# skokec/DAU-ConvNet

Measured on AMD Instinct MI355X. Metric: DAU fwd+bwd GSamples/s (N*H*W/s), higher is better.
Workload: dtype f32

## Files before the change

### dau-convnet_amd/csrc/dau_tiled.hpp

```cpp
#pragma once
#include "dau_common.hpp"

namespace dau {

struct TiledConfig {
    int N, Cin, Cout, G, H, W;
    int R;
    int blur_k;
    int NP;
    int windows;
    int stack;
    int patches;
    int rows, pitch;
    int tiles_x, tiles_y;
    int tile_w;
    int fblock;
    int variant;
    int debug;
    int act;
};

bool tiled_gather_configure(int N, int Cin, int Cout, int G, int H, int W, int R, int blur_k, int act, TiledConfig* cfg);
size_t tiled_gather_workspace_bytes(const TiledConfig& cfg);
int tiled_gather_windows(const TiledConfig& cfg);
// ... 10 lines not shown
    int ftiles;
};
#define DAU_DECLARE_DENSE_GATHER(NS)                                                                                           \
    namespace NS {                                                                                                            \
    bool dense_gather_configure(int N, int Cin, int Cout, int G, int H, int W, int R, int blur_k, int act, DenseConfig* cfg);  \
    size_t dense_gather_workspace_bytes(const DenseConfig& cfg);                                                              \
    void dense_gather_init(const DenseConfig& cfg);                                                                           \
      \
    void dense_gather_prepare(hipStream_t st, const DenseConfig& cfg, const float* in, const float* filters, bool mirrored,   \
                              const UnitRef* table, void* workspace, const Guard& guard);                                     \
    void dense_gather_run(hipStream_t st, const DenseConfig& cfg, float* out, void* workspace, const Guard& guard);           \
    }
DAU_DECLARE_DENSE_GATHER(r4)
DAU_DECLARE_DENSE_GATHER(r3)

#define DAU_DECLARE_SPLIT_GATHER(NS)                                                                                           \
    namespace NS {                                                                                                            \
    bool split_gather_configure(int N, int Cin, int Cout, int G, int H, int W, int R, int blur_k, int act, DenseConfig* cfg);  \
    size_t split_gather_workspace_bytes(const DenseConfig& cfg);                                                              \
    void split_gather_init(const DenseConfig& cfg);                                                                           \
    void split_gather_prepare(hipStream_t st, const DenseConfig& cfg, const float* in, const float* filters, bool mirrored,   \
                              const UnitRef* table, void* workspace, const Guard& guard);                                     \
    void split_gather_run(hipStream_t st, const DenseConfig& cfg, float* out, void* workspace, const Guard& guard);           \
    }
DAU_DECLARE_SPLIT_GATHER(s2)
DAU_DECLARE_SPLIT_GATHER(s3)
DAU_DECLARE_SPLIT_GATHER(s4)

struct TiledDotConfig {
    Shape sh;
    int R, blur_k;
    int NP;
    int variant;
    int windows;
    bool as1, one_tile;
    bool rw8;
    bool ring;
    int region_cols, region_rows;
    int rounds;
    int act;
    int ignore;
    int debug;
};

bool tiled_dot_configure(const Shape& sh, int R, int blur_k, int act, int ignore, TiledDotConfig* cfg);
size_t tiled_dot_workspace_bytes(const TiledDotConfig& cfg);
void tiled_dot_prepare(hipStream_t st, const TiledDotConfig& cfg, const float* x, const float* dy,
                       const float* filters, const UnitRef* table_bare, int drop_col, int drop_row, void* workspace,
                       const Guard& guard);
void tiled_dot_run(hipStream_t st, const TiledDotConfig& cfg, float* r4, void* workspace, const Guard& guard, bool accumulate);
void tiled_dot_init(const TiledDotConfig& cfg);

void launch_blur4_pack(hipStream_t st, const float* x, const float* filters, int N, int C, int cstride, int H, int W, int Hp,
                       int Wp, int blur_k, int act, float* xk, const Guard& guard);
void blur4_pack_init(int blur_k);
bool blur4_pack_fits(int blur_k, int Hp, int Wp);

void launch_dot_reduce(hipStream_t st, const void* partial, int partial_f32, long n, int G, int F, int g_split, int slabs0,
                       int slabs1, int zero_from, bool accumulate, float* r4, const Guard& guard);

struct SplitDotConfig {
    Shape sh;
    int blur_k;
    int RW;
    int act;
};
bool split_dot_configure(const Shape& sh, int blur_k, int act, SplitDotConfig* cfg);
size_t split_dot_workspace_bytes(const SplitDotConfig& cfg);
void split_dot_init(const SplitDotConfig& cfg);
void split_dot_prepare(hipStream_t st, const SplitDotConfig& cfg, const float* x, const float* dy, const float* filters,
                       int drop_col, int drop_row, void* workspace, const Guard& guard);
void split_dot_run(hipStream_t st, const SplitDotConfig& cfg, const UnitRef* table, float* r4, void* workspace, const Guard& guard);

struct WgradConfig {
    Shape sh;
    int blur_k;
    int SB, FB, NC;
    int HsT, WsT, WT, nseg;
    int splits;
    int Hp, Wp;
    bool fused;
};
#define DAU_DECLARE_DENSE_WGRAD(NS)                                                                                            \
    namespace NS {                                                                                                            \
    bool dense_wgrad_configure(const Shape& sh, int blur_k, bool bf16, WgradConfig* cfg);                                     \
    size_t dense_wgrad_workspace_bytes(const WgradConfig& cfg);                                                               \
    void dense_wgrad_init(const WgradConfig& cfg);                                                                            \
    void dense_wgrad_run(hipStream_t st, const WgradConfig& cfg, const float* x, const float* dy, const float* filters,       \
                         const UnitRef* table, int drop_col, int drop_row, float* r4, void* workspace, const Guard& guard, int nk); \
    }
DAU_DECLARE_DENSE_WGRAD(r4)
DAU_DECLARE_DENSE_WGRAD(r3)

}
```

### dau-convnet_amd/csrc/k_gather_dot.hip

```cpp
#include <cstdlib>
#include <algorithm>
#ifndef DAU_DOT_FLUSH_TERMS
#define DAU_DOT_FLUSH_TERMS 1024
#endif
#include <type_traits>
#include <utility>

#include "dau_tiled.hpp"

namespace dau {

typedef float f2 __attribute__((ext_vector_type(2)));
typedef float f4 __attribute__((ext_vector_type(4)));
typedef float f8 __attribute__((ext_vector_type(8)));
typedef float f16 __attribute__((ext_vector_type(16)));
typedef __attribute__((address_space(3))) void* lds_ptr_t;
typedef __attribute__((address_space(1))) const void* glb_ptr_t;

namespace {

constexpr int kDF = 32;
constexpr int kRW = 8;
#ifndef DAU_DOT_WAVES
#define DAU_DOT_WAVES 16
// ... 127 lines not shown
    const int nxc = (EX + kPackErrorChunk - 1) / kPackErrorChunk;
    int t0 = blockIdx.x;
    const int xc = t0 % nxc; t0 /= nxc;
    const int Y = t0 % EY; t0 /= EY;
    const int fb = t0 % nfb;
    const int np = t0 / nfb;
    const int y = Y - (R + 1);
    const int X0 = xc * kPackErrorChunk, X1 = X0 + kPackErrorChunk < EX ? X0 + kPackErrorChunk : EX;
    const int xa0 = X0 - (R + 1) > 0 ? X0 - (R + 1) : 0, xa1 = X1 - (R + 1) < W ? X1 - (R + 1) : W;
    const int cw = xa1 > xa0 ? xa1 - xa0 : 0;
    const int wp = (cw > 0 ? cw : 1) | 1;
    const bool rowin = y >= 0 && y < H && !(drop_row && y == H - 1);
    if (rowin && cw > 0) {
        auto fill = [&](auto actc) {
            constexpr int AF = decltype(actc)::value;
            const int total = 64 * cw;
            for (int t0 = threadIdx.x; t0 < total; t0 += blockDim.x * kLoadBatch) {
                typename RawAct<AF>::type v[kLoadBatch];
                int rr[kLoadBatch];
                bool okk[kLoadBatch];
#pragma unroll
                for (int u = 0; u < kLoadBatch; ++u) {
                    const int t = t0 + u * blockDim.x, tc = t < total ? t : total - 1;
                    const int r = tc / cw, x = tc - r * cw;
                    rr[u] = r;
                    const int f = fb * kDF + (r >> 1), n = 2 * np + (r & 1);
                    const bool ok = f < F && n < N;
                    const long src = (((long)(ok ? n : 0) * F + (ok ? f : 0)) * H + y) * W + xa0;
                    v[u] = load_raw<AF>(dy, src + x);
                    okk[u] = ok;
                }
#pragma unroll
                for (int u = 0; u < kLoadBatch; ++u) {
                    const int t = t0 + u * blockDim.x;
                    if (t < total) lds[rr[u] * wp + (t - rr[u] * cw)] = mask_act(act_of(v[u]), okk[u]);
                }
            }
        };
        with_act(act, fill);
    }
    __syncthreads();
    float* out = ep + ((((size_t)np * nfb + fb) * EY + Y) * EX + X0) * (kDF * 2);
    const int wlim = drop_col ? W - 1 : W;
    for (int t = threadIdx.x; t < (X1 - X0) * 64; t += blockDim.x) {
        const int X = X0 + (t >> 6), r = t & 63, x = X - (R + 1);
        out[t] = (rowin && x >= xa0 && x < xa1 && x < wlim) ? lds[r * wp + (x - xa0)] : 0.0f;
    }
}

struct Blur4Args {
    const float* in;
    const float* taps;
    float* xk;
    int N, C, cstride, H, W, k, Hp, Wp;
    int act;
    int ppb, items;
    unsigned lds_item_floats;
    int WY, WX, nwy, nwx;
    Guard guard;
};

template <int K>
__global__ void __launch_bounds__(512) blur4_pack_kernel(const Blur4Args a) {
    extern __shared__ __attribute__((aligned(16))) float lds[];
    if (!guard_pass(a.guard)) return;
    const int C = a.cstride, H = a.H, W = a.W, k = K ? K : a.k;
    const int Creal = a.C;
    const int lane = threadIdx.x & 63;
    const int nw = (blockDim.x >> 6) / a.ppb;
    const int sub = (threadIdx.x >> 6) / nw, wave = (threadIdx.x >> 6) % nw;
    int t = blockIdx.x * a.ppb + sub;
    const bool active = t < a.items;
    if (!active) t = a.items - 1;
    const int c = t % C; t /= C;
    const int wx = t % a.nwx; t /= a.nwx;
    const int wy = t % a.nwy;
    const int np = t / a.nwy;
    const int oy0 = wy * a.WY, ox0 = wx * a.WX;
    const int oh = oy0 + a.WY < a.Hp ? a.WY : a.Hp - oy0, ow = ox0 + a.WX < a.Wp ? a.WX : a.Wp - ox0;
    const int kr = (k - 1) / 2;
    const int lw = ow + 2 * kr, lh = oh + 2 * kr;
    f2* A = reinterpret_cast<f2*>(lds + (size_t)sub * a.lds_item_floats);
    f2* B = A + (size_t)lh * lw;
    const float* tp[6] = {a.taps + kTapGX * kTapPitch, a.taps + kTapAX * kTapPitch, a.taps + kTapCX * kTapPitch,
                          a.taps + kTapGY * kTapPitch, a.taps + kTapAY * kTapPitch, a.taps + kTapBY * kTapPitch};
    float tr[6][K ? K : 1];
    if (K) {
#pragma unroll
        for (int q = 0; q < 6; ++q)
#pragma unroll
            for (int i = 0; i < K; ++i) tr[q][i] = tp[q][i];
    }
    auto tap = [&](int q, int i) { return K ? tr[q][i] : tp[q][i]; };
    const int n0 = 2 * np, n1 = 2 * np + 1;
    const bool real = c < Creal;
    const int cs = real ? c : 0;
    const long p0 = ((long)n0 * Creal + cs) * H * W, p1 = ((long)(n1 < a.N ? n1 : n0) * Creal + cs) * H * W;
    const float m0 = real ? 1.0f : 0.0f;
    const float m1 = (real && n1 < a.N) ? 1.0f : 0.0f;
    auto for_each = [&](int rows_, int cols_, auto&& body) {
        if (cols_ >= 56) {
            for (int r = wave; r < rows_; r += nw)
                for (int x = lane; x < cols_; x += 64) body(r, x);
        } else {
            for (int t = wave * 64 + lane; t < rows_ * cols_; t += nw * 64) { const int r = t / cols_; body(r, t - r * cols_); }
        }
    };
    auto fill = [&](auto actc) {
        constexpr int AF = decltype(actc)::value;
        struct Raw2 { typename RawAct<AF>::type v0, v1; };
        load_phase<Raw2>(lh, lw, wave, nw, lane,
            [&](int r, int xl) {
                const int yy = oy0 - kr + r, xx = ox0 - kr + xl;
                const bool in = yy >= 0 && yy < H && xx >= 0 && xx < W;
                const long off = in ? (long)yy * W + xx : 0;
                return Raw2{load_raw<AF>(a.in, p0 + off), load_raw<AF>(a.in, p1 + off)};
            },
            [&](int r, int xl, Raw2 v) {
                const int yy = oy0 - kr + r, xx = ox0 - kr + xl;
                const bool in = yy >= 0 && yy < H && xx >= 0 && xx < W;
                A[r * lw + xl] = f2{mask_act(m0 * act_of(v.v0), in), mask_act(m1 * act_of(v.v1), in)};
            });
    };
    with_act(a.act, fill);
    __syncthreads();
    for_each(lh, ow, [&](int r, int x) {
        const int yy = oy0 - kr + r;
        f2 h1 = {0.0f, 0.0f}, h2 = {0.0f, 0.0f}, h3 = {0.0f, 0.0f};
        if (yy >= 0 && yy < H) {
#pragma unroll
            for (int i = 0; i < k; ++i) {
                const f2 v = A[r * lw + x + i];
                h1 = __builtin_elementwise_fma(v, f2{tap(0, i), tap(0, i)}, h1);
                h2 = __builtin_elementwise_fma(v, f2{tap(1, i), tap(1, i)}, h2);
                h3 = __builtin_elementwise_fma(v, f2{tap(2, i), tap(2, i)}, h3);
            }
        }
        B[(0 * lh + r) * ow + x] = h1; B[(1 * lh + r) * ow + x] = h2; B[(2 * lh + r) * ow + x] = h3;
    });
    __syncthreads();
    f8* out = reinterpret_cast<f8*>(a.xk) + ((size_t)np * a.cstride + c) * a.Hp * a.Wp;
    for_each(active ? oh : 0, ow, [&](int yr, int xc) {
        const int yy = oy0 + yr, xx = ox0 + xc;
        f2 dw = {0.0f, 0.0f}, d1 = {0.0f, 0.0f}, d2 = {0.0f, 0.0f}, ds = {0.0f, 0.0f};
        if (yy < H && xx < W) {
#pragma unroll
            for (int j = 0; j < k; ++j) {
                const f2 b1 = B[(0 * lh + yr + j) * ow + xc], b2 = B[(1 * lh + yr + j) * ow + xc], b3 = B[(2 * lh + yr + j) * ow + xc];
                dw = __builtin_elementwise_fma(b1, f2{tap(3, j), tap(3, j)}, dw);
                d1 = __builtin_elementwise_fma(b2, f2{tap(3, j), tap(3, j)}, d1);
                d2 = __builtin_elementwise_fma(b1, f2{tap(4, j), tap(4, j)}, d2);
                ds = __builtin_elementwise_fma(b3, f2{tap(3, j), tap(3, j)}, ds);
                ds = __builtin_elementwise_fma(b1, f2{tap(5, j), tap(5, j)}, ds);
            }
        }
        out[(size_t)yy * a.Wp + xx] = f8{dw.x, dw.y, d1.x, d1.y, d2.x, d2.y, ds.x, ds.y};
    });
}

__global__ void dot_params_kernel(const UnitRef* __restrict__ table, int S, int G, int F, int R, int Rt, int nsub1,
                                  int epitch, int g_begin, int GP, int ngb, int nfb, int s_pad, float* __restrict__ params,
                                  const Guard guard) {
    if (!guard_pass(guard)) return;
    const long total = (long)nsub1 * nsub1 * s_pad * ngb * GP * nfb * 64;
    for (long idx = blockIdx.x * (long)blockDim.x + threadIdx.x; idx < total; idx += (long)gridDim.x * blockDim.x) {
        const int lane = (int)(idx % 64);
        long t = idx / 64;
        const int fb = (int)(t % nfb); t /= nfb;
        const int gp = (int)(t % GP); t /= GP;
        const int gb = (int)(t % ngb); t /= ngb;
        const int s = (int)(t % s_pad);
        const int sub = (int)(t / s_pad);
        const int g = g_begin + gb * 2 * GP + 2 * gp + (lane >> 5), fl = lane & 31, f = fb * kDF + fl;
        UnitRef u{0, 0, 0.0f, 0.0f, 0.0f, 0.0f};
        if (s < S && g < G && f < F) u = table[((long)s * G + g) * F + f];
        int wy = (u.oy + R) / (2 * Rt), wx = (u.ox + R) / (2 * Rt);
        wy = wy < nsub1 ? wy : nsub1 - 1; wx = wx < nsub1 ? wx : nsub1 - 1;
        const int cy = -R + Rt + 2 * Rt * (sub / nsub1), cx = -R + Rt + 2 * Rt * (sub % nsub1);
        if (wy != sub / nsub1 || wx != sub % nsub1) u = UnitRef{cx, cy, 0.0f, 0.0f, 0.0f, 0.0f};
        const int base = (((Rt - (u.oy - cy)) * epitch + (Rt - (u.ox - cx))) * kDF + fl) * 8;
        float* dst = params + idx * kParamDwords;
        dst[0] = u.w00; dst[1] = u.w01; dst[2] = u.w10; dst[3] = u.w11;
        dst[4] = __int_as_float(base); dst[5] = 0.0f; dst[6] = 0.0f; dst[7] = 0.0f;
    }
}

constexpr int kWlMaxUnits = 16;

__global__ void __launch_bounds__(1024) dot_worklist_kernel(const UnitRef* __restrict__ table, int S, int G, int F, int R, int Rt,
                                                            int nsub1, int epitch, int nfb, int nsg, int sgroup, int rounds_max,
                                                            unsigned plane_bytes, float* __restrict__ params,
                                                            int* __restrict__ nrounds, const Guard guard) {
    if (!guard_pass(guard)) return;
    __shared__ int K[32], pre[32], hbase;
    __shared__ unsigned char cnt[32][32];
    __shared__ unsigned short where[32][32][kWlMaxUnits];
    __shared__ unsigned char mult[32][kWlMaxUnits][32];
    __shared__ unsigned char fill[32][kWlMaxUnits], degree[32][kWlMaxUnits];
    __shared__ int lane0_base[32][kWlMaxUnits];
    int t = blockIdx.x;
    const int sg = t % nsg; t /= nsg;
    const int fb = t % nfb;
    const int sub = t / nfb;
    const int fl = threadIdx.x & 31, sl = threadIdx.x >> 5;
    const int f = fb * kDF + fl;
    const int cy = -R + Rt + 2 * Rt * (sub / nsub1), cx = -R + Rt + 2 * Rt * (sub % nsub1);
    float* const pbase = params + (size_t)blockIdx.x * rounds_max * kWlSlots * 32 * kParamDwords;
    auto slot_ptr = [&](int h, int ln) -> float* {
        const int round = h / kWlSlots, hl = h % kWlSlots;
        const int wh = hl % (2 * kDWaves), entry = hl / (2 * kDWaves);
// ... 661 lines not shown
    const size_t s_pad = (size_t)g.s_pad;
    size_t off = 0;
    l.ep_off = off; off += round_up(NP * g.nfb * g.EY * g.EX * kDF * 8, 256);
    l.xk_off = off; off += round_up(NP * s_pad * g.Hp * g.Wp * 32 + (size_t)g.Wp * 32, 256);
    l.params_off = off;
    for (int i = 0; i < g.npass; ++i) off += g.pass[i].params_bytes;
    l.nrounds_off = off; off += round_up((size_t)g.nsub1 * g.nsub1 * g.nfb * g.pass[0].nsb * 4, 256);
    l.partial_off = off; off += round_up((size_t)g.chunks * kNumK * c.sh.S * c.sh.G * c.sh.F * 8, 256);
    l.total = off;
    return l;
}

void blur4_plan(int k, int Hp, int Wp, int* wy, int* wx, size_t* lds) {
    const int WX = Wp < 64 ? Wp : 64;
    auto bytes = [&](int WY) { return ((size_t)(WY + k - 1) * (WX + k - 1) + (size_t)3 * (WY + k - 1) * WX) * 8; };
    int WY = Hp;
    static const size_t limit = (size_t)DAU_TUNE_INT("DAU_BLUR4_LDS_KB", 74) * 1024;
    while (WY > 8 && bytes(WY) > limit) WY -= 8;
    *wy = WY; *wx = WX; *lds = bytes(WY);
}

template <int GP, int AS, int RH, bool BINNED = false, int RW = 8, bool RING = false>
void launch_dot(hipStream_t st, const DotArgs* a, int grid, size_t lds) {
    auto kern = gather_dot_kernel<GP, AS, RH, BINNED, RW, RING>;
    if (!a) { (void)hipFuncSetAttribute(reinterpret_cast<const void*>(kern), hipFuncAttributeMaxDynamicSharedMemorySize, 160 * 1024); return; }
    hipLaunchKernelGGL(kern, dim3(grid), dim3(kDWaves * 64), lds, st, *a);
}

void dispatch_dot(bool binned, bool ring, int RW, int RH, int GP, int AS, hipStream_t st, const DotArgs* a, int grid, size_t lds) {
    if (RW == 14) {
        if (AS == 2) launch_dot<2, 2, 4, false, 14>(st, a, grid, lds);
        else launch_dot<2, 1, 4, false, 14>(st, a, grid, lds);
        return;
    }
    if (binned) {
        if (ring) {
            if (RH == 8) launch_dot<1, 4, 8, true, 8, true>(st, a, grid, lds);
            else launch_dot<1, 4, 4, true, 8, true>(st, a, grid, lds);
            return;
        }
        if (RH == 8) launch_dot<1, 4, 8, true>(st, a, grid, lds);
        else launch_dot<1, 4, 4, true>(st, a, grid, lds);
    } else if (RH == 8) {
        if (GP == 1) launch_dot<1, 4, 8>(st, a, grid, lds);
        else if (AS == 2) launch_dot<2, 2, 8>(st, a, grid, lds);
        else launch_dot<2, 1, 8>(st, a, grid, lds);
    } else {
        if (GP == 1) launch_dot<1, 4, 7>(st, a, grid, lds);
        else if (AS == 2) launch_dot<2, 2, 7>(st, a, grid, lds);
        else launch_dot<2, 1, 7>(st, a, grid, lds);
    }
}

auto blur4_pack_for(int blur_k) {
    return blur_k == 7 ? blur4_pack_kernel<7> : blur_k == 5 ? blur4_pack_kernel<5> : blur_k == 9 ? blur4_pack_kernel<9> : blur4_pack_kernel<0>;
}

}

void launch_blur4_pack(hipStream_t st, const float* x, const float* filters, int N, int C, int cstride, int H, int W, int Hp,
                       int Wp, int blur_k, int act, float* xk, const Guard& guard) {
    int wy, wx; size_t blur_lds;
    blur4_plan(blur_k, Hp, Wp, &wy, &wx, &blur_lds);
    auto kern = blur4_pack_for(blur_k);
    Blur4Args b{};
    b.guard = guard;
    b.in = x; b.taps = filters + kTaps1dOffset; b.xk = xk;
    b.N = N; b.C = C; b.cstride = cstride; b.H = H; b.W = W; b.k = blur_k; b.Hp = Hp; b.Wp = Wp; b.act = act;
    b.WY = wy; b.WX = wx; b.nwy = (Hp + wy - 1) / wy; b.nwx = (Wp + wx - 1) / wx;
    const int elems = wy * wx;
    b.ppb = elems >= 2048 ? 1 : elems >= 1024 ? 2 : elems >= 512 ? 4 : 8;
    while (b.ppb > 1 && b.ppb * blur_lds > 64 * 1024) b.ppb /= 2;
    b.items = ((N + 1) / 2) * b.nwy * b.nwx * cstride;
    b.lds_item_floats = (unsigned)(blur_lds / 4);
    hipLaunchKernelGGL(kern, dim3((b.items + b.ppb - 1) / b.ppb), dim3(512), b.ppb * blur_lds, st, b);
}
void launch_dot_reduce(hipStream_t st, const void* partial, int partial_f32, long n, int G, int F, int g_split, int slabs0,
                       int slabs1, int zero_from, bool accumulate, float* r4, const Guard& guard) {
    const int rgrid = (int)((n + 255) / 256 < 4096 ? (n + 255) / 256 : 4096);
    hipLaunchKernelGGL(dot_reduce_kernel, dim3(rgrid), dim3(256), 0, st, partial, partial_f32, n, G, F, g_split, slabs0, slabs1,
                       zero_from, accumulate ? 1 : 0, r4, guard);
}
void blur4_pack_init(int blur_k) {
    (void)hipFuncSetAttribute(reinterpret_cast<const void*>(blur4_pack_for(blur_k)), hipFuncAttributeMaxDynamicSharedMemorySize, 160 * 1024);
}
bool blur4_pack_fits(int blur_k, int Hp, int Wp) {
    int wy, wx; size_t blur_lds;
    blur4_plan(blur_k, Hp, Wp, &wy, &wx, &blur_lds);
    return blur_lds <= 150 * 1024;
}

bool tiled_dot_configure(const Shape& sh, int R, int blur_k, int act, int ignore, TiledDotConfig* cfg) {
    const bool as1 = DAU_TUNE_SET("DAU_DOT_AS1");
    const bool one_tile = DAU_TUNE_INT("DAU_DOT_NBUF", 2) == 1;
    const int rounds = DAU_TUNE_INT("DAU_DOT_ROUNDS", 0);
    const bool rw8 = DAU_TUNE_INT("DAU_DOT_RW", 0) == 8;
    const DotGeometry g = make_dot_geometry(sh, R, as1, one_tile, rounds, rw8);
    if (g.nbuf * g.tile_bytes > 160 * 1024) return false;
    if (g.nsub1 > 1 && g.sgroup == 0) return false;
    if (g.nsub1 > 1 && sh.G > kWlMaxUnits) return false;
    if ((size_t)g.epitch * kDF * 8 + (g.RW + 1) * kDF * 8 > 65535) return false;
    {
        int wy, wx; size_t blur_lds;
        blur4_plan(blur_k, g.Hp, g.Wp, &wy, &wx, &blur_lds);
        if (blur_lds > 150 * 1024) return false;
    }
    TiledDotConfig c{};
    c.sh = sh; c.R = R; c.blur_k = blur_k; c.NP = (sh.N + 1) / 2; c.variant = g.npass; c.windows = g.nsub1 * g.nsub1;
    c.act = act; c.ignore = ignore;
    c.ring = g.nsub1 > 1 && g.nbuf == 1 && DAU_TUNE_INT("DAU_DOT_RING", 1) != 0;
    c.as1 = as1; c.one_tile = one_tile; c.rounds = rounds; c.rw8 = rw8; c.region_cols = g.RW; c.region_rows = g.RH; c.debug = DAU_TUNE_INT("DAU_DOT_DEBUG", 0);
    *cfg = c;
    return true;
}

size_t tiled_dot_workspace_bytes(const TiledDotConfig& c) {
    return dot_layout(c, make_dot_geometry(c.sh, c.R, c.as1, c.one_tile, c.rounds, c.rw8)).total;
}

void tiled_dot_init(const TiledDotConfig& c) {
    const DotGeometry g = make_dot_geometry(c.sh, c.R, c.as1, c.one_tile, c.rounds, c.rw8);
    for (int i = 0; i < g.npass; ++i) dispatch_dot(g.nsub1 > 1, c.ring, g.RW, g.RH, g.pass[i].GP, g.pass[i].AS, nullptr, nullptr, 0, 0);
    (void)hipFuncSetAttribute(reinterpret_cast<const void*>(pack_error_kernel), hipFuncAttributeMaxDynamicSharedMemorySize, 160 * 1024);
    (void)hipFuncSetAttribute(reinterpret_cast<const void*>(blur4_pack_for(c.blur_k)), hipFuncAttributeMaxDynamicSharedMemorySize, 160 * 1024);
}

void tiled_dot_prepare(hipStream_t st, const TiledDotConfig& c, const float* x, const float* dy, const float* filters,
                       const UnitRef* table_bare, int drop_col, int drop_row, void* workspace, const Guard& guard) {
    const DotGeometry g = make_dot_geometry(c.sh, c.R, c.as1, c.one_tile, c.rounds, c.rw8);
    const DotLayout l = dot_layout(c, g);
    char* ws = static_cast<char*>(workspace);
    const Shape& s = c.sh;
    const int s_pad = g.s_pad;
    {
        const int cwmax = s.W < kPackErrorChunk ? s.W : kPackErrorChunk;
        const size_t lds = (size_t)64 * (cwmax | 1) * 4;
        const int nxc = (g.EX + kPackErrorChunk - 1) / kPackErrorChunk;
        hipLaunchKernelGGL(pack_error_kernel, dim3(c.NP * g.nfb * g.EY * nxc), dim3(256), lds, st, dy, s.N, s.F, s.H, s.W, g.Rp, g.EX,
                           g.EY, g.nfb, drop_col, drop_row, c.act, reinterpret_cast<float*>(ws + l.ep_off), guard);
    }
    launch_blur4_pack(st, x, filters, s.N, s.S, s_pad, s.H, s.W, g.Hp, g.Wp, c.blur_k, c.act, reinterpret_cast<float*>(ws + l.xk_off), guard);
    if (g.nsub1 > 1) {
        const DotGeometry::Pass& ps = g.pass[0];
        hipLaunchKernelGGL(dot_worklist_kernel, dim3(g.nsub1 * g.nsub1 * g.nfb * ps.nsb), dim3(1024), 0, st, table_bare, s.S, s.G, s.F,
                           g.Rp, g.Rt, g.nsub1, g.epitch, g.nfb, ps.nsb, g.sgroup, ps.ngb, (unsigned)((size_t)g.Hp * g.Wp * 32),
                           reinterpret_cast<float*>(ws + l.params_off + ps.params_off), reinterpret_cast<int*>(ws + l.nrounds_off), guard);
        return;
    }
    for (int i = 0; i < g.npass; ++i) {
        const DotGeometry::Pass& ps = g.pass[i];
        const long total = (long)g.nsub1 * g.nsub1 * s_pad * ps.ngb * ps.GP * g.nfb * 64;
        const int grid = (int)((total + 255) / 256 < 4096 ? (total + 255) / 256 : 4096);
        hipLaunchKernelGGL(dot_params_kernel, dim3(grid), dim3(256), 0, st, table_bare, s.S, s.G, s.F, g.Rp, g.Rt, g.nsub1,
                           g.epitch, ps.g_begin, ps.GP, ps.ngb, g.nfb, s_pad,
                           reinterpret_cast<float*>(ws + l.params_off + ps.params_off), guard);
    }
}

void tiled_dot_run(hipStream_t st, const TiledDotConfig& c, float* r4, void* workspace, const Guard& guard, bool accumulate) {
    const DotGeometry g = make_dot_geometry(c.sh, c.R, c.as1, c.one_tile, c.rounds, c.rw8);
    const DotLayout l = dot_layout(c, g);
    char* ws = static_cast<char*>(workspace);
    const Shape& s = c.sh;
    DotArgs a{};
    a.ep = ws + l.ep_off;
    a.xk = reinterpret_cast<const float*>(ws + l.xk_off);
    a.partial = ws + l.partial_off;
    a.N = s.N; a.S = s.S; a.F = s.F; a.G = s.G; a.R = g.Rp;
    a.NP = c.NP; a.nfb = g.nfb; a.nbuf = g.nbuf; a.Rt = g.Rt; a.nsub1 = g.nsub1; a.chunks = g.chunks; a.items = g.items;
    a.rx = g.rx; a.ry = g.ry; a.EX = g.EX; a.EY = g.EY; a.Hp = g.Hp; a.Wp = g.Wp; a.epitch = g.epitch; a.erows = g.erows;
    a.s_pad = g.s_pad;
    a.nrounds = reinterpret_cast<const int*>(ws + l.nrounds_off);
    a.sgroup = g.sgroup;
    a.tile_bytes = (unsigned)g.tile_bytes;
    a.debug = c.debug;
    a.guard = guard;
    const bool binned = g.nsub1 > 1;
// ... 28 lines not shown
```

### dau-convnet_amd/csrc/k_split_dot.hip

```cpp
#include <algorithm>
#include <cfloat>

#include "dau_tiled.hpp"

namespace dau {

typedef _Float16 h8 __attribute__((ext_vector_type(8)));
typedef float f4s __attribute__((ext_vector_type(4)));

namespace {

constexpr int kSdWaves = 8;
constexpr int kSdAS = 2;
constexpr int kSdGT = 4;
constexpr int kSdSB = kSdWaves * kSdAS;
constexpr int kSdFB = 16;
constexpr int kSdR = 4;
constexpr int kSdRH = 4;
constexpr int kSdFlushItems = 16;
constexpr unsigned kVmcnt0 = 0x0F70, kVmcnt8 = 0x0F78;

inline size_t rup(size_t v, size_t a = 256) { return (v + a - 1) / a * a; }

struct SdGeom {
    int Hq, Wq, rq, cq, XTr, XTc, EYs, EXs, octs, nfb, nsb, ngb, items, chunks, per, NP;
};

SdGeom sd_geom(const SplitDotConfig& c) {
    const Shape& s = c.sh;
    SdGeom g{};
    g.Hq = (s.H + 1 + kSdRH - 1) / kSdRH * kSdRH;
    g.Wq = (s.W + 1 + c.RW - 1) / c.RW * c.RW;
    g.rq = g.Hq / kSdRH; g.cq = g.Wq / c.RW;
    g.XTr = g.Hq + 1; g.XTc = g.Wq + 1;
    g.EYs = g.Hq + 2 * kSdR; g.EXs = g.Wq + 2 * kSdR;
    g.octs = (s.N + 7) / 8;
    g.NP = (s.N + 1) / 2;
    g.nfb = (s.F + kSdFB - 1) / kSdFB;
    g.nsb = (s.S + kSdSB - 1) / kSdSB;
    g.ngb = (s.G + kSdGT - 1) / kSdGT;
    g.items = g.octs * g.rq * g.cq;
    const int per_chunk = g.nfb * g.nsb * g.ngb;
    int chunks = (1024 + per_chunk - 1) / per_chunk;
    chunks = std::max(1, std::min(chunks, g.items));
    g.per = (g.items + chunks - 1) / chunks;
    g.chunks = (g.items + g.per - 1) / g.per;
    return g;
}

struct SdLayout { size_t maxes_off, xk_off, xs_off, es_off, partial_off, total; };

SdLayout sd_layout(const SplitDotConfig& c, const SdGeom& g) {
    const Shape& s = c.sh;
    SdLayout l{};
    size_t off = 0;
    l.maxes_off = off; off += rup((size_t)(s.S * kNumK + s.F) * 4);
    l.xk_off = off; off += rup((size_t)g.NP * s.S * s.H * s.W * 32);
    l.xs_off = off; off += rup((size_t)g.octs * s.S * kNumK * g.XTr * g.XTc * 32 + 32);
    l.es_off = off; off += rup((size_t)g.octs * g.nfb * g.EYs * g.EXs * 512);
    l.partial_off = off; off += rup((size_t)g.chunks * kNumK * s.S * s.G * s.F * 4);
    l.total = off;
    return l;
}

__device__ __forceinline__ int sd_shift(unsigned maxbits) {
    if (maxbits == 0u) return 0;
    const int e = (int)(maxbits >> 23) - 127;
    const int sh = 13 - e;
    return sh > 120 ? 120 : sh;
}

__device__ __forceinline__ bool finite_abs(float v, float* a) {
    *a = fabsf(v);
    return *a <= FLT_MAX;
}

__global__ void __launch_bounds__(256) sd_absmax_x_kernel(const float* __restrict__ xk, int NP, int S, int HW, int split,
                                                          unsigned* __restrict__ xmax, const Guard guard) {
    if (!guard_pass(guard)) return;
    const int s = blockIdx.x % S, part = blockIdx.x / S;
    float m[4] = {0.0f, 0.0f, 0.0f, 0.0f};
    const long per_np = (long)HW * 2;
    const long total = (long)NP * per_np;
    for (long i = part * 256L + threadIdx.x; i < total; i += 256L * split) {
        const long np = i / per_np, r = i - np * per_np;
        const float4 v = reinterpret_cast<const float4*>(xk + ((size_t)np * S + s) * HW * 8)[r];
        const int k0 = (int)(r & 1) * 2;
        float a;
        if (finite_abs(v.x, &a)) m[k0] = fmaxf(m[k0], a);
        if (finite_abs(v.y, &a)) m[k0] = fmaxf(m[k0], a);
        if (finite_abs(v.z, &a)) m[k0 + 1] = fmaxf(m[k0 + 1], a);
        if (finite_abs(v.w, &a)) m[k0 + 1] = fmaxf(m[k0 + 1], a);
    }
    __shared__ float red[4][256];
    for (int k = 0; k < 4; ++k) red[k][threadIdx.x] = m[k];
    __syncthreads();
    for (int w = 128; w >= 1; w >>= 1) {
        if ((int)threadIdx.x < w)
            for (int k = 0; k < 4; ++k) red[k][threadIdx.x] = fmaxf(red[k][threadIdx.x], red[k][threadIdx.x + w]);
        __syncthreads();
    }
    if (threadIdx.x < 4) atomicMax(&xmax[s * kNumK + threadIdx.x], __float_as_uint(red[threadIdx.x][0]));
}

__global__ void __launch_bounds__(256) sd_absmax_e_kernel(const float* __restrict__ dy, int N, int F, int HW, int split, int act,
                                                          unsigned* __restrict__ emax, const Guard guard) {
    if (!guard_pass(guard)) return;
    const int f = blockIdx.x % F, part = blockIdx.x / F;
    float m = 0.0f;
    const long total = (long)N * HW;
    for (long i = part * 256L + threadIdx.x; i < total; i += 256L * split) {
        const long n = i / HW, p = i - n * HW;
        float a;
        if (finite_abs(load_act(dy, ((long)n * F + f) * HW + p, act), &a)) m = fmaxf(m, a);
    }
    for (int o = 32; o >= 1; o >>= 1) m = fmaxf(m, __shfl_xor(m, o));
    if ((threadIdx.x & 63) == 0) atomicMax(&emax[f], __float_as_uint(m));
}

__device__ __forceinline__ void split_limbs(float v, _Float16* hi, _Float16* lo) {
    const _Float16 h = (_Float16)v;
    const float hf = (float)h;
    *hi = h;
    *lo = (hf - hf == 0.0f) ? (_Float16)(v - hf) : (_Float16)0.0f;
}

__global__ void __launch_bounds__(256) sd_stage_x_kernel(const float* __restrict__ xk, const unsigned* __restrict__ xmax, int N,
                                                         int NP, int S, int H, int W, int octs, int XTr, int XTc,
                                                         h8* __restrict__ xs, const Guard guard) {
    if (!guard_pass(guard)) return;
    const long total = (long)octs * S * XTr * XTc;
    for (long idx = blockIdx.x * 256L + threadIdx.x; idx < total; idx += (long)gridDim.x * 256) {
        long t = idx;
        const int tx = (int)(t % XTc); t /= XTc;
        const int ty = (int)(t % XTr); t /= XTr;
        const int s = (int)(t % S);
        const int oct = (int)(t / S);
        const int y = ty - 1, x = tx - 1;
        const bool in = y >= 0 && y < H && x >= 0 && x < W;
        float v[4][8];
#pragma unroll
        for (int p = 0; p < 4; ++p) {
            const int np = oct * 4 + p;
            float4 a = make_float4(0.f, 0.f, 0.f, 0.f), b = a;
            if (in && np < NP) {
                const float4* src = reinterpret_cast<const float4*>(xk + ((((size_t)np * S + s) * H + y) * W + x) * 8);
                a = src[0]; b = src[1];
            }
            v[0][2 * p] = a.x; v[0][2 * p + 1] = a.y; v[1][2 * p] = a.z; v[1][2 * p + 1] = a.w;
            v[2][2 * p] = b.x; v[2][2 * p + 1] = b.y; v[3][2 * p] = b.z; v[3][2 * p + 1] = b.w;
        }
#pragma unroll
        for (int k = 0; k < 4; ++k) {
            const float sc = ldexpf(1.0f, sd_shift(xmax[s * kNumK + k]));
            h8 hi, lo;
#pragma unroll
            for (int i = 0; i < 8; ++i) {
                _Float16 h, l;
                split_limbs(v[k][i] * sc, &h, &l);
                hi[i] = h; lo[i] = l;
            }
            h8* dst = xs + ((((size_t)oct * S + s) * kNumK + k) * XTr * XTc + (size_t)ty * XTc + tx) * 2;
            dst[0] = hi; dst[1] = lo;
        }
    }
}

__global__ void __launch_bounds__(256) sd_stage_e_kernel(const float* __restrict__ dy, const unsigned* __restrict__ emax, int N,
                                                         int F, int H, int W, int octs, int nfb, int EYs, int EXs, int drop_col,
                                                         int drop_row, int act, h8* __restrict__ es, const Guard guard) {
    if (!guard_pass(guard)) return;
    const long total = (long)octs * nfb * EYs * EXs;
    const int wlim = drop_col ? W - 1 : W, hlim = drop_row ? H - 1 : H;
    for (long idx = blockIdx.x * 256L + threadIdx.x; idx < total; idx += (long)gridDim.x * 256) {
        long t = idx;
        const int vx = (int)(t % EXs); t /= EXs;
        const int vy = (int)(t % EYs); t /= EYs;
        const int fb = (int)(t % nfb);
        const int oct = (int)(t / nfb);
        const int y = vy - (kSdR + 1), x = vx - (kSdR + 1);
        const bool in = y >= 0 && y < hlim && x >= 0 && x < wlim;
        h8* dst = es + (size_t)idx * 32;
        for (int fl = 0; fl < kSdFB; ++fl) {
            const int f = fb * kSdFB + fl;
            const float sc = f < F ? ldexpf(1.0f, sd_shift(emax[f])) : 0.0f;
            h8 hi, lo;
#pragma unroll
            for (int i = 0; i < 8; ++i) {
                const int n = oct * 8 + i;
                const float v = (in && f < F && n < N) ? load_act(dy, (((long)n * F + f) * H + y) * W + x, act) : 0.0f;
                _Float16 h, l;
                split_limbs(v * sc, &h, &l);
                hi[i] = h; lo[i] = l;
            }
            dst[fl] = hi; dst[kSdFB + fl] = lo;
        }
    }
}

struct SdArgs {
    const h8* xs;
    const char* es;
    const unsigned* xmax;
    const unsigned* emax;
    const UnitRef* table;
    float* partial;
    int S, F, G;
    int nfb, nsb, ngb, per, items, rq, cq, XTr, XTc, EYs, EXs;
    Guard guard;
};

__device__ __forceinline__ void sd_glds16(const char* src, unsigned dst) {
    unsigned keep;
    asm volatile("s_mov_b32 %0, m0\n\ts_mov_b32 m0, %2\n\ts_nop 0\n\tglobal_load_lds_dwordx4 %1, off\n\ts_mov_b32 m0, %0"
                 : "=&s"(keep) : "v"(src), "s"(dst) : "memory");
}

#ifndef DAU_SD_STEP_LOADS
__device__ __forceinline__ h8 sd_next_col(h8 cur, h8 nxt, int dx) {
    typedef int i4s __attribute__((ext_vector_type(4)));
    const i4s c = __builtin_bit_cast(i4s, cur), n = __builtin_bit_cast(i4s, nxt);
    i4s r;
#pragma unroll
    for (int d = 0; d < 4; ++d)
        r[d] = __builtin_amdgcn_update_dpp(0, dx ? c[d] : n[d], 0xB1 , 0xF, 0xF, true);
    return __builtin_bit_cast(h8, r);
}
#endif

template <int RW>
__global__ void __launch_bounds__(kSdWaves * 64) __attribute__((amdgpu_waves_per_eu(2, 2))) split_gather_dot_kernel(const SdArgs a) {
    extern __shared__ __attribute__((aligned(16))) char lds[];
    if (!guard_pass(a.guard)) return;
    constexpr int WL = RW + 2 * kSdR, WR = kSdRH + 2 * kSdR;
    constexpr int kRing = WR + kSdRH;
    constexpr unsigned RB = WL * 512;
    constexpr int kRowPieces = (RB + 1023) / 1024;
    static_assert((kRing & (kRing - 1)) == 0, "ring slot = (origin + row) & (kRing - 1)");
    static_assert(RW % 2 == 0, "A fragment sets by the parity of the K step / of the pair of K steps");
#ifdef DAU_SD_STEP_LOADS
    constexpr int kSdAStride = 2;
#else
    constexpr int kSdAStride = 4;
#endif
    static_assert((size_t)kRing * RB <= 160 * 1024, "the ring fills the LDS");
    int t = blockIdx.x;
    const int gb = t % a.ngb; t /= a.ngb;
    const int sb = t % a.nsb; t /= a.nsb;
    const int fb = t % a.nfb; t /= a.nfb;
    const int chunk = t;
    const int it0 = chunk * a.per, it1 = min(it0 + a.per, a.items);
// ... 190 lines not shown
            for (int gg = 0; gg < kSdGT; ++gg) {
                const int g = gb * kSdGT + gg;
                const bool ok = s_ok[i] && g < a.G && f_ok;
                const f4s p = part[i][gg], w = wb[i][gg];
                float v = w[0] * p[0];
                v = fmaf(w[1], p[1], v);
                v = fmaf(w[2], p[2], v);
                v = fmaf(w[3], p[3], v);
                run[i][gg] += ok ? v : 0.0f;
            }
        if (++since_flush == kSdFlushItems) { flush(); since_flush = 0; }
    }
    asm volatile("s_waitcnt vmcnt(0)" ::: "memory");
    if (since_flush) flush();
}

template <int RW>
void launch_sd(hipStream_t st, const SdArgs* a, int grid) {
    auto kern = split_gather_dot_kernel<RW>;
    const size_t lds = (size_t)(2 * kSdRH + 2 * kSdR) * (RW + 2 * kSdR) * 512;
    if (!a) { (void)hipFuncSetAttribute(reinterpret_cast<const void*>(kern), hipFuncAttributeMaxDynamicSharedMemorySize, 160 * 1024); return; }
    hipLaunchKernelGGL(kern, dim3(grid), dim3(kSdWaves * 64), lds, st, *a);
}
void dispatch_sd(int RW, hipStream_t st, const SdArgs* a, int grid) {
    if (RW == 10) launch_sd<10>(st, a, grid);
    else launch_sd<12>(st, a, grid);
}

}

bool split_dot_configure(const Shape& sh, int blur_k, int act, SplitDotConfig* cfg) {
    if (act == kActBF16) return false;
    int best = 0;
    long best_cost = 1L << 40;
    for (int rw = 12; rw >= 10; rw -= 2) {
        const long wq = (sh.W + 1 + rw - 1) / rw * rw;
        const long cost = wq * (rw + 2) * (60 / rw);
        if (cost < best_cost) { best_cost = cost; best = rw; }
    }
    if ((size_t)(2 * kSdRH + 2 * kSdR) * (best + 2 * kSdR) * 512 > 160 * 1024) return false;
    if (!blur4_pack_fits(blur_k, sh.H, sh.W)) return false;
    SplitDotConfig c{};
    c.sh = sh; c.blur_k = blur_k; c.RW = best; c.act = act;
    const SdGeom g = sd_geom(c);
    if ((long)g.EXs * 512 * 32 > (1L << 31)) return false;
    *cfg = c;
    return true;
}

size_t split_dot_workspace_bytes(const SplitDotConfig& c) { return sd_layout(c, sd_geom(c)).total; }

void split_dot_init(const SplitDotConfig& c) {
    dispatch_sd(c.RW, nullptr, nullptr, 0);
    blur4_pack_init(c.blur_k);
}

void split_dot_prepare(hipStream_t st, const SplitDotConfig& c, const float* x, const float* dy, const float* filters,
                       int drop_col, int drop_row, void* workspace, const Guard& guard) {
    const SdGeom g = sd_geom(c);
    const SdLayout l = sd_layout(c, g);
    const Shape& s = c.sh;
    char* ws = static_cast<char*>(workspace);
    unsigned* xmax = reinterpret_cast<unsigned*>(ws + l.maxes_off);
    unsigned* emax = xmax + s.S * kNumK;
    float* xk = reinterpret_cast<float*>(ws + l.xk_off);
    (void)hipMemsetAsync(xmax, 0, (size_t)(s.S * kNumK + s.F) * 4, st);
    (void)hipMemsetAsync(ws + l.partial_off, 0, (size_t)g.chunks * kNumK * s.S * s.G * s.F * 4, st);
    launch_blur4_pack(st, x, filters, s.N, s.S, s.S, s.H, s.W, s.H, s.W, c.blur_k, c.act, xk, guard);
    const int HW = s.H * s.W;
    const int xsplit = std::max(1, std::min(16, 2048 / std::max(1, s.S)));
    hipLaunchKernelGGL(sd_absmax_x_kernel, dim3(s.S * xsplit), dim3(256), 0, st, xk, g.NP, s.S, HW, xsplit, xmax, guard);
    const int esplit = std::max(1, std::min(16, 2048 / std::max(1, s.F)));
    hipLaunchKernelGGL(sd_absmax_e_kernel, dim3(s.F * esplit), dim3(256), 0, st, dy, s.N, s.F, HW, esplit, c.act, emax, guard);
    hipLaunchKernelGGL(sd_stage_x_kernel, dim3(8192), dim3(256), 0, st, xk, xmax, s.N, g.NP, s.S, s.H, s.W, g.octs, g.XTr, g.XTc,
                       reinterpret_cast<h8*>(ws + l.xs_off), guard);
    hipLaunchKernelGGL(sd_stage_e_kernel, dim3(4096), dim3(256), 0, st, dy, emax, s.N, s.F, s.H, s.W, g.octs, g.nfb, g.EYs, g.EXs,
                       drop_col, drop_row, c.act, reinterpret_cast<h8*>(ws + l.es_off), guard);
}

void split_dot_run(hipStream_t st, const SplitDotConfig& c, const UnitRef* table, float* r4, void* workspace, const Guard& guard) {
    const SdGeom g = sd_geom(c);
    const SdLayout l = sd_layout(c, g);
    const Shape& s = c.sh;
    char* ws = static_cast<char*>(workspace);
    SdArgs a{};
    a.xs = reinterpret_cast<const h8*>(ws + l.xs_off);
    a.es = ws + l.es_off;
    a.xmax = reinterpret_cast<const unsigned*>(ws + l.maxes_off);
    a.emax = a.xmax + s.S * kNumK;
    a.table = table;
    a.partial = reinterpret_cast<float*>(ws + l.partial_off);
    a.S = s.S; a.F = s.F; a.G = s.G;
    a.nfb = g.nfb; a.nsb = g.nsb; a.ngb = g.ngb; a.per = g.per; a.items = g.items; a.rq = g.rq; a.cq = g.cq;
    a.XTr = g.XTr; a.XTc = g.XTc; a.EYs = g.EYs; a.EXs = g.EXs;
    a.guard = guard;
    dispatch_sd(c.RW, st, &a, g.chunks * g.nfb * g.nsb * g.ngb);
    launch_dot_reduce(st, a.partial, 1, (long)kNumK * s.S * s.G * s.F, s.G, s.F, s.G, g.chunks, g.chunks, s.G, false, r4, guard);
}

}
```

Measured before the change: 0.01566.

## Fuse x abs-max into blur pack and tile the error staging kernel

The blur4 pack kernel now optionally computes per-channel abs-max of the four packed derivative planes, using a wave reduction plus atomicMax, so the separate sd_absmax_x pass over xk is no longer launched. The dy staging kernel is rewritten to give each block one row segment of one filter block. It splits values into fp16 hi/lo limbs into an XOR-swizzled LDS tile and writes coalesced h8 rows, with zero padding handled per column. This removes a full read of xk and aims to improve memory coalescing of the staging writes, at the cost of extra atomics and register use in the pack kernel. The old path stays available behind DAU_SD_STAGE_REF.

```diff
diff --git a/dau-convnet_amd/csrc/dau_tiled.hpp b/dau-convnet_amd/csrc/dau_tiled.hpp
--- a/dau-convnet_amd/csrc/dau_tiled.hpp
+++ b/dau-convnet_amd/csrc/dau_tiled.hpp
@@ -86,8 +86,8 @@
 void tiled_dot_init(const TiledDotConfig& cfg);
 
 void launch_blur4_pack(hipStream_t st, const float* x, const float* filters, int N, int C, int cstride, int H, int W, int Hp,
-                       int Wp, int blur_k, int act, float* xk, const Guard& guard);
-void blur4_pack_init(int blur_k);
+                       int Wp, int blur_k, int act, float* xk, const Guard& guard, unsigned* kmax = nullptr);
+void blur4_pack_init(int blur_k, bool kmax = false);
 bool blur4_pack_fits(int blur_k, int Hp, int Wp);
 
 void launch_dot_reduce(hipStream_t st, const void* partial, int partial_f32, long n, int G, int F, int g_split, int slabs0,
diff --git a/dau-convnet_amd/csrc/k_gather_dot.hip b/dau-convnet_amd/csrc/k_gather_dot.hip
--- a/dau-convnet_amd/csrc/k_gather_dot.hip
+++ b/dau-convnet_amd/csrc/k_gather_dot.hip
@@ -203,6 +203,7 @@
     const float* in;
     const float* taps;
     float* xk;
+    unsigned* kmax;
     int N, C, cstride, H, W, k, Hp, Wp;
     int act;
     int ppb, items;
@@ -211,7 +212,7 @@
     Guard guard;
 };
 
-template <int K>
+template <int K, bool KMAX>
 __global__ void __launch_bounds__(512) blur4_pack_kernel(const Blur4Args a) {
     extern __shared__ __attribute__((aligned(16))) float lds[];
     if (!guard_pass(a.guard)) return;
@@ -291,6 +292,12 @@
     });
     __syncthreads();
     f8* out = reinterpret_cast<f8*>(a.xk) + ((size_t)np * a.cstride + c) * a.Hp * a.Wp;
+    constexpr unsigned kKeyZero = 1u << 24;
+    unsigned km[4] = {kKeyZero, kKeyZero, kKeyZero, kKeyZero}, seen[4] = {0u, 0u, 0u, 0u};
+    if constexpr (KMAX) {
+#pragma unroll
+        for (int q = 0; q < 4; ++q) seen[q] = __hip_atomic_load(a.kmax + c * kNumK + q, __ATOMIC_RELAXED, __HIP_MEMORY_SCOPE_AGENT);
+    }
     for_each(active ? oh : 0, ow, [&](int yr, int xc) {
         const int yy = oy0 + yr, xx = ox0 + xc;
         f2 dw = {0.0f, 0.0f}, d1 = {0.0f, 0.0f}, d2 = {0.0f, 0.0f}, ds = {0.0f, 0.0f};
@@ -306,7 +313,22 @@
             }
         }
         out[(size_t)yy * a.Wp + xx] = f8{dw.x, dw.y, d1.x, d1.y, d2.x, d2.y, ds.x, ds.y};
+        if constexpr (KMAX) {
+            const f2 kv[4] = {dw, d1, d2, ds};
+#pragma unroll
+            for (int q = 0; q < 4; ++q)
+                km[q] = max(max(km[q], (__float_as_uint(kv[q].x) << 1) + kKeyZero), (__float_as_uint(kv[q].y) << 1) + kKeyZero);
+        }
     });
+    if constexpr (KMAX) {
+#pragma unroll
+        for (int q = 0; q < 4; ++q) {
+            unsigned m = km[q];
+            for (int o = 32; o >= 1; o >>= 1) m = max(m, (unsigned)__shfl_xor((int)m, o));
+            const unsigned bits = (m - kKeyZero) >> 1;
+            if (lane == 0 && bits > seen[q]) atomicMax(a.kmax + c * kNumK + q, bits);
+        }
+    }
 }
 
 __global__ void dot_params_kernel(const UnitRef* __restrict__ table, int S, int G, int F, int R, int Rt, int nsub1,
@@ -1074,20 +1096,24 @@
     }
 }
 
-auto blur4_pack_for(int blur_k) {
-    return blur_k == 7 ? blur4_pack_kernel<7> : blur_k == 5 ? blur4_pack_kernel<5> : blur_k == 9 ? blur4_pack_kernel<9> : blur4_pack_kernel<0>;
-}
+template <bool KMAX>
+const void* blur4_pack_pick(int blur_k) {
+    auto kern = blur_k == 7 ? blur4_pack_kernel<7, KMAX> : blur_k == 5 ? blur4_pack_kernel<5, KMAX>
+              : blur_k == 9 ? blur4_pack_kernel<9, KMAX> : blur4_pack_kernel<0, KMAX>;
+    return reinterpret_cast<const void*>(kern);
+}
+const void* blur4_pack_for(int blur_k, bool kmax = false) { return kmax ? blur4_pack_pick<true>(blur_k) : blur4_pack_pick<false>(blur_k); }
 
 }
 
 void launch_blur4_pack(hipStream_t st, const float* x, const float* filters, int N, int C, int cstride, int H, int W, int Hp,
-                       int Wp, int blur_k, int act, float* xk, const Guard& guard) {
+                       int Wp, int blur_k, int act, float* xk, const Guard& guard, unsigned* kmax) {
     int wy, wx; size_t blur_lds;
     blur4_plan(blur_k, Hp, Wp, &wy, &wx, &blur_lds);
-    auto kern = blur4_pack_for(blur_k);
+    const void* kern = blur4_pack_for(blur_k, kmax != nullptr);
     Blur4Args b{};
     b.guard = guard;
-    b.in = x; b.taps = filters + kTaps1dOffset; b.xk = xk;
+    b.in = x; b.taps = filters + kTaps1dOffset; b.xk = xk; b.kmax = kmax;
     b.N = N; b.C = C; b.cstride = cstride; b.H = H; b.W = W; b.k = blur_k; b.Hp = Hp; b.Wp = Wp; b.act = act;
     b.WY = wy; b.WX = wx; b.nwy = (Hp + wy - 1) / wy; b.nwx = (Wp + wx - 1) / wx;
     const int elems = wy * wx;
@@ -1095,7 +1121,8 @@
     while (b.ppb > 1 && b.ppb * blur_lds > 64 * 1024) b.ppb /= 2;
     b.items = ((N + 1) / 2) * b.nwy * b.nwx * cstride;
     b.lds_item_floats = (unsigned)(blur_lds / 4);
-    hipLaunchKernelGGL(kern, dim3((b.items + b.ppb - 1) / b.ppb), dim3(512), b.ppb * blur_lds, st, b);
+    void* params[] = {&b};
+    (void)hipLaunchKernel(kern, dim3((b.items + b.ppb - 1) / b.ppb), dim3(512), params, b.ppb * blur_lds, st);
 }
 void launch_dot_reduce(hipStream_t st, const void* partial, int partial_f32, long n, int G, int F, int g_split, int slabs0,
                        int slabs1, int zero_from, bool accumulate, float* r4, const Guard& guard) {
@@ -1103,8 +1130,8 @@
     hipLaunchKernelGGL(dot_reduce_kernel, dim3(rgrid), dim3(256), 0, st, partial, partial_f32, n, G, F, g_split, slabs0, slabs1,
                        zero_from, accumulate ? 1 : 0, r4, guard);
 }
-void blur4_pack_init(int blur_k) {
-    (void)hipFuncSetAttribute(reinterpret_cast<const void*>(blur4_pack_for(blur_k)), hipFuncAttributeMaxDynamicSharedMemorySize, 160 * 1024);
+void blur4_pack_init(int blur_k, bool kmax) {
+    (void)hipFuncSetAttribute(blur4_pack_for(blur_k, kmax), hipFuncAttributeMaxDynamicSharedMemorySize, 160 * 1024);
 }
 bool blur4_pack_fits(int blur_k, int Hp, int Wp) {
     int wy, wx; size_t blur_lds;
@@ -1144,7 +1171,7 @@
     const DotGeometry g = make_dot_geometry(c.sh, c.R, c.as1, c.one_tile, c.rounds, c.rw8);
     for (int i = 0; i < g.npass; ++i) dispatch_dot(g.nsub1 > 1, c.ring, g.RW, g.RH, g.pass[i].GP, g.pass[i].AS, nullptr, nullptr, 0, 0);
     (void)hipFuncSetAttribute(reinterpret_cast<const void*>(pack_error_kernel), hipFuncAttributeMaxDynamicSharedMemorySize, 160 * 1024);
-    (void)hipFuncSetAttribute(reinterpret_cast<const void*>(blur4_pack_for(c.blur_k)), hipFuncAttributeMaxDynamicSharedMemorySize, 160 * 1024);
+    (void)hipFuncSetAttribute(blur4_pack_for(c.blur_k), hipFuncAttributeMaxDynamicSharedMemorySize, 160 * 1024);
 }
 
 void tiled_dot_prepare(hipStream_t st, const TiledDotConfig& c, const float* x, const float* dy, const float* filters,
diff --git a/dau-convnet_amd/csrc/k_split_dot.hip b/dau-convnet_amd/csrc/k_split_dot.hip
--- a/dau-convnet_amd/csrc/k_split_dot.hip
+++ b/dau-convnet_amd/csrc/k_split_dot.hip
@@ -75,6 +75,7 @@
     return *a <= FLT_MAX;
 }
 
+#ifdef DAU_SD_STAGE_REF
 __global__ void __launch_bounds__(256) sd_absmax_x_kernel(const float* __restrict__ xk, int NP, int S, int HW, int split,
                                                           unsigned* __restrict__ xmax, const Guard guard) {
     if (!guard_pass(guard)) return;
@@ -102,6 +103,7 @@
     }
     if (threadIdx.x < 4) atomicMax(&xmax[s * kNumK + threadIdx.x], __float_as_uint(red[threadIdx.x][0]));
 }
+#endif
 
 __global__ void __launch_bounds__(256) sd_absmax_e_kernel(const float* __restrict__ dy, int N, int F, int HW, int split, int act,
                                                           unsigned* __restrict__ emax, const Guard guard) {
@@ -166,6 +168,54 @@
     }
 }
 
+#ifndef DAU_SD_STAGE_REF
+constexpr int kSeTX = 80;
+__global__ void __launch_bounds__(256) sd_stage_e_kernel(const float* __restrict__ dy, const unsigned* __restrict__ emax, int N,
+                                                         int F, int H, int W, int nfb, int EYs, int EXs, int nct, int TX,
+                                                         int drop_col, int drop_row, int act, h8* __restrict__ es,
+                                                         const Guard guard) {
+    __shared__ h8 tile[kSeTX * 32];
+    if (!guard_pass(guard)) return;
+    int t = blockIdx.x;
+    const int ct = t % nct; t /= nct;
+    const int vy = t % EYs; t /= EYs;
+    const int fb = t % nfb;
+    const int oct = t / nfb;
+    const int wlim = drop_col ? W - 1 : W, hlim = drop_row ? H - 1 : H;
+    const int vx0 = ct * TX, nvx = min(TX, EXs - vx0);
+    const int y = vy - (kSdR + 1);
+    const int c0 = max(vx0, kSdR + 1), c1 = (y >= 0 && y < hlim) ? min(vx0 + nvx, kSdR + 1 + wlim) : c0;
+    const int nd = max(c1 - c0, 0);
+    for (int i = threadIdx.x; i < kSdFB * nd; i += 256) {
+        const int fl = i / nd, vx = c0 + (i - fl * nd), x = vx - (kSdR + 1), lx = vx - vx0;
+        const int f = fb * kSdFB + fl;
+        const float sc = f < F ? ldexpf(1.0f, sd_shift(emax[f])) : 0.0f;
+        float v[8];
+#pragma unroll
+        for (int n = 0; n < 8; ++n) {
+            const int img = oct * 8 + n;
+            v[n] = (f < F && img < N) ? load_act(dy, (((long)img * F + f) * H + y) * W + x, act) : 0.0f;
+        }
+        h8 hi, lo;
+#pragma unroll
+        for (int n = 0; n < 8; ++n) {
+            _Float16 h, l;
+            split_limbs(v[n] * sc, &h, &l);
+            hi[n] = h; lo[n] = l;
+        }
+        tile[lx * 32 + (fl ^ (lx & 7))] = hi;
+        tile[lx * 32 + ((kSdFB + fl) ^ (lx & 7))] = lo;
+    }
+    if (nd > 0) __syncthreads();
+    h8* dst = es + ((((size_t)oct * nfb + fb) * EYs + vy) * EXs + vx0) * 32;
+    for (int q = threadIdx.x; q < nvx * 32; q += 256) {
+        const int lx = q >> 5, vx = vx0 + lx;
+        h8 piece = {0, 0, 0, 0, 0, 0, 0, 0};
+        if (vx >= c0 && vx < c1) piece = tile[lx * 32 + ((q & 31) ^ (lx & 7))];
+        dst[q] = piece;
+    }
+}
+#else
 __global__ void __launch_bounds__(256) sd_stage_e_kernel(const float* __restrict__ dy, const unsigned* __restrict__ emax, int N,
                                                          int F, int H, int W, int octs, int nfb, int EYs, int EXs, int drop_col,
                                                          int drop_row, int act, h8* __restrict__ es, const Guard guard) {
@@ -197,6 +247,7 @@
         }
     }
 }
+#endif
 
 struct SdArgs {
     const h8* xs;
@@ -493,7 +544,11 @@
 
 void split_dot_init(const SplitDotConfig& c) {
     dispatch_sd(c.RW, nullptr, nullptr, 0);
+#ifndef DAU_SD_STAGE_REF
+    blur4_pack_init(c.blur_k, true);
+#else
     blur4_pack_init(c.blur_k);
+#endif
 }
 
 void split_dot_prepare(hipStream_t st, const SplitDotConfig& c, const float* x, const float* dy, const float* filters,
@@ -507,16 +562,26 @@
     float* xk = reinterpret_cast<float*>(ws + l.xk_off);
     (void)hipMemsetAsync(xmax, 0, (size_t)(s.S * kNumK + s.F) * 4, st);
     (void)hipMemsetAsync(ws + l.partial_off, 0, (size_t)g.chunks * kNumK * s.S * s.G * s.F * 4, st);
+    const int HW = s.H * s.W;
+#ifndef DAU_SD_STAGE_REF
+    launch_blur4_pack(st, x, filters, s.N, s.S, s.S, s.H, s.W, s.H, s.W, c.blur_k, c.act, xk, guard, xmax);
+#else
     launch_blur4_pack(st, x, filters, s.N, s.S, s.S, s.H, s.W, s.H, s.W, c.blur_k, c.act, xk, guard);
-    const int HW = s.H * s.W;
     const int xsplit = std::max(1, std::min(16, 2048 / std::max(1, s.S)));
     hipLaunchKernelGGL(sd_absmax_x_kernel, dim3(s.S * xsplit), dim3(256), 0, st, xk, g.NP, s.S, HW, xsplit, xmax, guard);
+#endif
     const int esplit = std::max(1, std::min(16, 2048 / std::max(1, s.F)));
     hipLaunchKernelGGL(sd_absmax_e_kernel, dim3(s.F * esplit), dim3(256), 0, st, dy, s.N, s.F, HW, esplit, c.act, emax, guard);
     hipLaunchKernelGGL(sd_stage_x_kernel, dim3(8192), dim3(256), 0, st, xk, xmax, s.N, g.NP, s.S, s.H, s.W, g.octs, g.XTr, g.XTc,
                        reinterpret_cast<h8*>(ws + l.xs_off), guard);
+#ifndef DAU_SD_STAGE_REF
+    const int nct = (g.EXs + kSeTX - 1) / kSeTX, tx = (g.EXs + nct - 1) / nct;
+    hipLaunchKernelGGL(sd_stage_e_kernel, dim3((unsigned)(g.octs * g.nfb * g.EYs * nct)), dim3(256), 0, st, dy, emax, s.N, s.F, s.H,
+                       s.W, g.nfb, g.EYs, g.EXs, nct, tx, drop_col, drop_row, c.act, reinterpret_cast<h8*>(ws + l.es_off), guard);
+#else
     hipLaunchKernelGGL(sd_stage_e_kernel, dim3(4096), dim3(256), 0, st, dy, emax, s.N, s.F, s.H, s.W, g.octs, g.nfb, g.EYs, g.EXs,
                        drop_col, drop_row, c.act, reinterpret_cast<h8*>(ws + l.es_off), guard);
+#endif
 }
 
 void split_dot_run(hipStream_t st, const SplitDotConfig& c, const UnitRef* table, float* r4, void* workspace, const Guard& guard) {
```

Result: faster. 0.01599 (median of 6 runs) (+2.1%).
